# flo-stilz/Audio-Key-Estimation

Hardware: AMD Instinct MI355X
Metric: clips/s (15 s @ 22.05 kHz), HIP CQT + PitchClassNet forward (higher is better)
Workload: dtype f32 accumulation everywhere; pitch / semitone / layer-0 convolutions: f16 activations x f16 weights (per-channel power-of-two scaled) on MFMA, one product; last layer's pitch-class convolutions and heads: 3-term split-bf16 on MFMA (hi*hi + lo*hi + hi*lo); CQT filter bank: 3-term split-bf16 on MFMA

## Files before the change

### audio-key-estimation_amd/csrc/pcnet.hip

```cpp
#include <algorithm>
#include <cmath>
#include <cstdlib>
#include <cstring>
#include <map>
#include <string>
#include <vector>

#include "common.h"
#include "pcnet_kernels.h"
#include "pcnet_bwd_kernels.h"

using namespace ake_k;

namespace {

constexpr double kBnEps = 1e-5;
constexpr size_t kLdsBudget = 64 * 1024;
constexpr size_t kBfFragsPerConv = 14 * 2 * 64 + 64;

struct TensorSpec {
    std::string name;
    int64_t shape[4];
    int ndim;
};
// ... 2273 lines not shown
                                  "conv_p2p_f16x3_kernel/p2p", nullptr, true)) {
                    sdesc = Src{out, d.out_p, nullptr, 0, 0};
                    continue;
                }
                if ((rc = conv(n->p2p[i][j], train ? n->p2p_t[i][j] : n->p2p[i][j], m + "p2p.layer." + std::to_string(3 * j + 1), 0, sdesc,
                               in_aff, B, P, Ti, true, out, d.out_p, 0, out_aff, "conv_mfma_kernel/p2p")))
                    return rc;
                sdesc = Src{out, d.out_p, nullptr, 0, 0};
                in_aff = out_aff;
            }
            if (fused_fold) {
            } else if (fused_semi) {
                if ((rc = run_fold_max(out, d.out_p, P / 3, B, Ti, cat, ctot, d.prev_pc, s))) return rc;
            } else if (c.stay_sixth && train) {
                const long long total = static_cast<long long>(B) * d.out_p * 12 * Ti;
                ake::ProfScope ps("fold_affine_kernel", s);
                hipLaunchKernelGGL(fold_affine_kernel, dim3(static_cast<unsigned>((total + 255) / 256)), dim3(256), 0, s, out, out_aff, cat, d.out_p, P / 12, Ti,
                                   ctot, d.prev_pc, total);
                identity(b.aff_cat[i] + 3 * d.prev_pc, d.out_p);
            } else if (c.stay_sixth) {
                if ((rc = fold_maps(i, out, d.out_p, P, B, Ti, cat, ctot, d.prev_pc))) return rc;
            } else if ((rc = semi(i, out, out_aff, B, P, Ti, cat, ctot, d.prev_pc, train ? b.aff_cat[i] + 3 * d.prev_pc : nullptr))) return rc;
            if (last) return AKE_OK;
            const float* psrc = cat;
            const float* psrc_aff = train ? b.aff_cat[i] : nullptr;
            int cin = ctot;
            float* pdst = nullptr;
            float* pdst_aff = nullptr;
            if (c.resblock && train) {
                if ((rc = res_stack_train(n->pc2pc_t[i], m + "pc2pc.layer.", 1, Src{psrc, cin, nullptr, 0, 0}, psrc_aff, B, 12, Ti, b.pcst[i], b.aff_pcst[i],
                                          nullptr, 0, "conv_mfma_kernel/pc2pc")))
                    return rc;
                pdst = b.pcst[i].back(); pdst_aff = b.aff_pcst[i].back();
            } else if (c.resblock) {
                if ((rc = res_stack(n->pc2pc[i], 1, Src{psrc, cin, nullptr, 0, 0}, B, 12, Ti, b.pca[i], b.pcb[i], nullptr, 0, "conv_mfma_kernel/pc2pc"))) return rc;
                pdst = b.pca[i];
            }
            for (int j = 0; j < c.conv_layers && !c.resblock; ++j) {
                pdst = train ? b.pcst[i][j] : ((j & 1) ? b.pcb[i] : b.pca[i]);
                pdst_aff = !train ? nullptr : b.aff_pcst[i][j];
                if ((rc = conv(n->pc2pc[i][j], train ? n->pc2pc_t[i][j] : n->pc2pc[i][j], m + "pc2pc.layer." + std::to_string(3 * j + 1), 1,
                               Src{psrc, cin, nullptr, 0, 0}, psrc_aff, B, 12, Ti, true, pdst, d.out_pc, 0, pdst_aff, "conv_mfma_kernel/pc2pc")))
                    return rc;
                psrc = pdst; psrc_aff = pdst_aff; cin = d.out_pc;
            }
            const LayerDims& dn = n->dims[i + 1];
            const int ctn = dn.prev_pc + dn.out_p;
            const int Tn = Ti / tp;
            float* catn = b.cat[i + 1] + (i + 1 == L - 1 ? static_cast<size_t>(c0) * ctn * 12 * Tn : 0);
            time_pool(pdst, pdst_aff, B, d.out_pc, 12, Ti, catn, ctn, 0);
            if (train) identity(b.aff_cat[i + 1], d.out_pc);
            time_pool(out, out_aff, B, d.out_p, P, Ti, b.ppool[i], d.out_p, 0);
            pc_cur = catn; p_cur = b.ppool[i]; cp = d.out_p;
        }
        return AKE_OK;
    }

    int tail(int B, const int64_t* seq, float* key_out, float* tonic_out, float* genre_out) {
        const auto& c = n->cfg;
        const int L = c.num_layers, tp = c.time_pool_size;
        const int i = L - 1;
        const int Ti = b.Tl[i];
        const LayerDims& d = n->dims[i];
        int rc;
        const float* psrc = L == 1 ? b.fold0 : b.cat[i];
        const float* psrc_aff = (train && L > 1) ? b.aff_cat[i] : nullptr;
        int cin = L == 1 ? 1 : d.prev_pc + d.out_p;
        const int cout_default = L == 1 ? c.n_filters : d.out_pc;
        const int cout = cout_default;
        const std::string m = "model." + std::to_string(i) + ".pc2pc.layer.";
        float* pdst = nullptr;
        float* pdst_aff = nullptr;
        const bool pc_bf = !train && pc2pc_uses_bf16(n, i, Ti);
        const bool head_bf = !train && L > 1 && n->final_ch == 16 && c.head_layers >= 2 && n->head_key[0].bf_off >= 0 &&
                             n->head_tonic[0].bf_off >= 0 && b.Tf <= kPcBf16MaxFrames;
        const bool pc_fused = !train && L > 1 && !c.denseblock && pc2pc_fuses(n, i, Ti);
        if (pc_fused) {
            if ((rc = run_pc2pc_fused(n, i, psrc, cin, B, Ti, b.pcf, head_bf ? b.feat_cl : nullptr, s))) return rc;
        } else if (pc_bf) run_nchw_to_cl16(psrc, cin, B, Ti, reinterpret_cast<unsigned short*>(b.pcb[i]), s);
        if (c.resblock && train) {
            if ((rc = res_stack_train(n->pc2pc_t[i], m, 1, Src{psrc, cin, nullptr, 0, 0}, psrc_aff, B, 12, Ti, b.pcst[i], b.aff_pcst[i], nullptr, 0,
                                      L == 1 ? "conv_mfma_kernel/pc2pc0" : "conv_mfma_kernel/pc2pc")))
                return rc;
            pdst = b.pcst[i].back(); pdst_aff = b.aff_pcst[i].back();
        } else if (c.resblock) {
            if ((rc = res_stack(n->pc2pc[i], 1, Src{psrc, cin, nullptr, 0, 0}, B, 12, Ti, b.pca[i], b.pcb[i], nullptr, 0,
                                L == 1 ? "conv_mfma_kernel/pc2pc0" : "conv_mfma_kernel/pc2pc")))
                return rc;
            pdst = b.pca[i];
        }
        if (c.denseblock) {
            float* feat_buf = L == 1 ? b.fold0 : b.cat[i];
            if (train) {
                if ((rc = dense_stack_train(n->dense_pc[i], 1, feat_buf, n->final_ch, cin, B, 12, Ti, b.dn_bott_pc[i], b.dn_aff1_pc[i], b.dn_aff2_pc[i],
                                            L == 1 ? "conv_mfma_kernel/pc2pc0" : "conv_mfma_kernel/pc2pc")))
                    return rc;
            } else if ((rc = dense_stack(n->dense_pc[i], 1, feat_buf, n->final_ch, cin, B, 12, Ti, b.pca[i],
                                         L == 1 ? "conv_mfma_kernel/pc2pc0" : "conv_mfma_kernel/pc2pc")))
                return rc;
            pdst = feat_buf; pdst_aff = nullptr;
        }
        for (int j = 0; j < c.conv_layers && !pc_fused && !c.resblock && !c.denseblock; ++j) {
            pdst = train ? b.pcst[i][j] : ((j & 1) ? b.pcb[i] : b.pca[i]);
            pdst_aff = !train ? nullptr : b.aff_pcst[i][j];
            if (pc_bf) {
                const bool last_conv = j == c.conv_layers - 1;
                const unsigned short* in = reinterpret_cast<const unsigned short*>((j & 1) ? b.pca[i] : b.pcb[i]);
                if ((rc = run_pc_bf16(n, n->pc2pc[i][j], in, B, Ti, true, true, last_conv ? pdst : nullptr,
                                      last_conv ? nullptr : reinterpret_cast<unsigned short*>(pdst), s, "conv_pc_bf16_kernel/pc2pc")))
                    return rc;
                continue;
            }
            if (train && L > 1 && pc_f16x3_ok(n->pc2pc_t[i][j], Ti, true)) {
                const PackedConv& pt = n->pc2pc_t[i][j];
                unsigned short* planes = reinterpret_cast<unsigned short*>(b.pcb[i]);
                run_nchw_to_cl16_f16x2(psrc, cin, B, Ti, psrc_aff, planes, s);
                const int bn = bn_of(m + std::to_string(3 * j + 1));
                if ((rc = run_pc_bf16(n, pt, planes, B, Ti, true, false, pdst, nullptr, s, "conv_pc_f16x3_kernel/pc2pc", nullptr, nullptr, true,
                                      b.stats + 2 * n->bns[bn].ch_off, 2 * n->bn_channels)))
                    return rc;
                finalize_bn(bn, static_cast<double>(B) * 12 * Ti, pdst_aff);
                psrc = pdst; psrc_aff = pdst_aff; cin = cout;
                continue;
            }
            if ((rc = conv(n->pc2pc[i][j], train ? n->pc2pc_t[i][j] : n->pc2pc[i][j], m + std::to_string(3 * j + 1), 1,
                           Src{psrc, cin, nullptr, 0, 0}, psrc_aff, B, 12, Ti, true, pdst, cout, 0, pdst_aff,
                           L == 1 ? "conv_mfma_kernel/pc2pc0" : "conv_mfma_kernel/pc2pc")))
                return rc;
            psrc = pdst; psrc_aff = pdst_aff; cin = cout;
        }
        const float* feat = pdst;
        const float* feat_aff = pdst_aff;
        if (pc_fused) { feat = b.pcf; feat_aff = nullptr; }
        else if (L > 1) {
            const int cout = c.denseblock ? n->final_ch : cout_default;
            time_pool(pdst, pdst_aff, B, cout, 12, Ti, b.pcf, cout, 0);
            feat = b.pcf; feat_aff = nullptr;
        }
        const int Tf = b.Tf;
        struct HeadRun { const std::vector<PackedConv>* ce; const std::vector<PackedConv>* ct; float* hid; float* map; int kind; const char* nm; };
        HeadRun heads[3] = {{&n->head_key, &n->head_key_t, b.hid_k, b.map_k, 1, "key_classifier"},
                            {&n->head_tonic, &n->head_tonic_t, b.hid_t, b.map_t, 1, "tonic_classifier"},
                            {&n->head_genre, &n->head_genre_t, b.hid_g, b.map_g, 2, "genre_classifier"}};
        int Tm = Tf;
        bool head_planes_ready = false;
        int pooled_heads = 0;
        unsigned short* feat_cl = b.feat_cl;
        if (head_bf && !pc_fused) run_nchw_to_cl16(feat, n->final_ch, B, Tf, feat_cl, s);
        const int T1 = Tf - (c.kernel_size - 1), T2 = T1 - (c.kernel_size - 1);
        const bool head1_bf = head_bf && c.head_layers == 2 && n->head_key[1].bf_off >= 0 && n->head_tonic[1].bf_off >= 0 && T2 > 0 &&
                              (12 * ((T2 + 15) / 16) + 15) / 16 <= kHead1MT;
        const bool genre_bf = head1_bf && c.genre && n->head_genre.size() == 2 && n->head_genre[0].bf_off >= 0 && n->head_genre[1].bf_off >= 0 &&
                              n->head_genre[0].kh == 1 && n->head_genre[1].kh == 2;
        if (head1_bf) {
            Head1BfArgs ha;
            std::memset(&ha, 0, sizeof(ha));
            float* maps[3] = {b.map_k, b.map_t, b.map_g};
            float* hids[3] = {b.hid_k, b.hid_t, b.hid_g};
            const PackedConv* c0[3] = {&n->head_key[0], &n->head_tonic[0], genre_bf ? &n->head_genre[0] : nullptr};
            const PackedConv* c1[3] = {&n->head_key[1], &n->head_tonic[1], genre_bf ? &n->head_genre[1] : nullptr};
            const int nh = genre_bf ? 3 : 2;
            for (int h = 0; h < nh; ++h) {
                unsigned short* planes = reinterpret_cast<unsigned short*>(hids[h]);
                if (h == 0 && (rc = run_pc_bf16(n, *c0[0], feat_cl, B, Tf, false, true, nullptr, planes, s, "conv_pc_bf16_kernel/head", c0[1],
                                                reinterpret_cast<unsigned short*>(hids[1]))))
                    return rc;
                if (h == 2 && (rc = run_pc_bf16(n, *c0[h], feat_cl, B, Tf, false, true, nullptr, planes, s, "conv_pc_bf16_kernel/genre_head")))
                    return rc;
                ha.xh[h] = planes; ha.xl[h] = planes + static_cast<long long>(B) * 12 * T1 * 32;
                ha.bfrag[h] = n->bf_frags_dev + c1[h]->bf_off; ha.bias[h] = n->blob_dev + c1[h]->b_off; ha.dst[h] = maps[h];
                ha.KH[h] = c1[h]->kh; ha.circular[h] = c1[h]->kh == 12 ? 1 : 0; ha.H_out[h] = ha.circular[h] ? 12 : 12 - c1[h]->kh + 1;
            }
            ha.T_in = T1; ha.T_out = T2; ha.JB = (T2 + 15) / 16; ha.Tp = 16 * (ha.JB - 1) + 22;
            size_t lds = std::max(static_cast<size_t>(2) * 12 * ha.Tp * 4 * sizeof(uint4), static_cast<size_t>(8) * kHead1MT * 4 * 64 * sizeof(float));
            if (c.local == 0) {
                ha.fin_off = static_cast<int>(lds / sizeof(float));
                lds += static_cast<size_t>(12) * T2 * sizeof(float);
                float* outs[3] = {key_out, tonic_out, genre_out};
                for (int h = 0; h < nh; ++h) ha.pout[h] = outs[h];
                ha.seq = reinterpret_cast<const long long*>(seq);
                ha.n_pool_layers = L - 1; ha.tp = tp; ha.shrink = (c.kernel_size - 1) * c.head_layers; ha.max_pool = c.max_pool; ha.clip0 = 0;
                pooled_heads = nh;
            }
            static ake::DeviceOnce h1_attr;
            if (h1_attr.need()) {
                AKE_HIP_CHECK(hipFuncSetAttribute(reinterpret_cast<const void*>(conv_head1_bf16_kernel), hipFuncAttributeMaxDynamicSharedMemorySize, 150 * 1024));
                h1_attr.mark();
            }
            AKE_REQUIRE(lds <= 150 * 1024, AKE_ERR_UNSUPPORTED, "heads: %d frames do not fit conv_head1_bf16_kernel", T1);
            ake::ProfScope ps("conv_head1_bf16_kernel", s);
            hipLaunchKernelGGL(conv_head1_bf16_kernel, dim3(B, nh), dim3(512), lds, s, ha);
            Tm = T2;
        }
        for (int h = head1_bf ? (genre_bf ? 3 : 2) : 0; h < (c.genre ? 3 : 2); ++h) {
            const float* src = feat;
            const float* src_aff = feat_aff;
            int hc = n->final_ch, Tcur = Tf;
            const size_t hid_half = static_cast<size_t>(B) * 2 * n->final_ch * 12 * Tf;
            for (int j = 0; j < c.head_layers; ++j) {
                const PackedConv& pe = (*heads[h].ce)[j];
                const bool lastj = j == c.head_layers - 1;
                float* dst = lastj ? heads[h].map : (train ? b.hst[h][j] : heads[h].hid + (j & 1) * hid_half);
                float* aff = (!train || lastj) ? nullptr : b.aff_hst[h][j];
                if (head_bf && h < 2 && j == 0) {
                    if ((rc = run_pc_bf16(n, pe, feat_cl, B, Tcur, false, true, dst, nullptr, s, "conv_pc_bf16_kernel/head"))) return rc;
                    src = dst; src_aff = aff; hc = pe.cout; Tcur -= c.kernel_size - 1;
                    continue;
                }
                if (train && j == 0 && !lastj && pc_f16x3_ok((*heads[h].ct)[0], Tcur, false)) {
                    const PackedConv& pt = (*heads[h].ct)[0];
                    if (!head_planes_ready) {
                        run_nchw_to_cl16_f16x2(src, hc, B, Tcur, src_aff, b.feat_cl, s);
                        head_planes_ready = true;
                    }
                    const int bn = bn_of(std::string(heads[h].nm) + ".1");
                    if ((rc = run_pc_bf16(n, pt, b.feat_cl, B, Tcur, false, false, dst, nullptr, s,
                                          h == 2 ? "conv_pc_f16x3_kernel/genre_head" : "conv_pc_f16x3_kernel/head", nullptr, nullptr, true,
                                          b.stats + 2 * n->bns[bn].ch_off, 2 * n->bn_channels)))
                        return rc;
                    const int H_out = heads[h].kind == 2 ? 12 - pt.kh + 1 : 12;
                    finalize_bn(bn, static_cast<double>(B) * H_out * (Tcur - pt.kw + 1), aff);
                    src = dst; src_aff = aff; hc = pe.cout; Tcur -= c.kernel_size - 1;
                    continue;
                }
                if (train && lastj && j > 0 && pe.cout == 1 && pe.kw == 7 && !n->raw_w_off.empty()) {
                    const std::string wn = std::string(heads[h].nm) + "." + std::to_string(3 * j) + (heads[h].kind == 2 ? "" : ".conv2d");
                    const auto wi = n->spec_index.find(wn + ".weight"), bi = n->spec_index.find(wn + ".bias");
                    const size_t lds = (static_cast<size_t>(hc) * 12 * Tcur + static_cast<size_t>(hc) * pe.kh * 7) * sizeof(float);
                    if (wi != n->spec_index.end() && bi != n->spec_index.end() && lds <= 150 * 1024 && Tcur - 6 >= 1) {
                        static ake::DeviceOnce hl_attr;
                        if (hl_attr.need()) {
                            AKE_HIP_CHECK(hipFuncSetAttribute(reinterpret_cast<const void*>(conv_head_last_kernel), hipFuncAttributeMaxDynamicSharedMemorySize, 150 * 1024));
                            hl_attr.mark();
                        }
                        ake::ProfScope ps(h == 2 ? "conv_head_last_kernel/genre" : "conv_head_last_kernel", s);
                        hipLaunchKernelGGL(conv_head_last_kernel, dim3(B), dim3(384), lds, s, src, src_aff, n->blob_dev + n->raw_w_off[wi->second],
                                           n->blob_dev + n->raw_w_off[bi->second], dst, hc, pe.kh, heads[h].kind == 2 ? 0 : 1, Tcur, Tcur - 6);
                        src = dst; src_aff = aff; hc = pe.cout; Tcur -= c.kernel_size - 1;
                        continue;
                    }
                }
                if ((rc = conv(pe, train ? (*heads[h].ct)[j] : pe, lastj ? "" : std::string(heads[h].nm) + "." + std::to_string(3 * j + 1),
                               heads[h].kind, Src{src, hc, nullptr, 0, 0}, src_aff, B, 12, Tcur, false, dst, pe.cout, 0, aff,
                               h == 2 ? "conv_mfma_kernel/genre_head" : "conv_mfma_kernel/head")))
                    return rc;
                src = dst; src_aff = aff; hc = pe.cout; Tcur -= c.kernel_size - 1;
            }
            Tm = Tcur;
        }
        if (c.local > 0) {
            AKE_REQUIRE(Tm >= c.local, AKE_ERR_INVALID, "pcnet --local: %d map frames are fewer than the pooling window %d", Tm, c.local);
            LocalPoolArgs la;
            std::memset(&la, 0, sizeof(la));
            la.maps[0] = b.map_k; la.maps[1] = b.map_t; la.maps[2] = c.genre ? b.map_g : nullptr;
            la.outs[0] = key_out; la.outs[1] = tonic_out; la.outs[2] = genre_out;
            la.Tm = Tm; la.Tq = Tm - c.local + 1; la.W = c.local; la.batch = B;
            ake::ProfScope ps("local_pool_kernel", s);
            hipLaunchKernelGGL(local_pool_kernel, dim3(static_cast<unsigned>((static_cast<long long>(B) * 12 * Tm + 255) / 256), 3), dim3(256), 0, s, la);
            AKE_HIP_CHECK(hipGetLastError());
            return AKE_OK;
        }
        PoolHeadArgs pa;
        std::memset(&pa, 0, sizeof(pa));
        pa.maps[0] = b.map_k; pa.maps[1] = b.map_t; pa.maps[2] = c.genre ? b.map_g : nullptr;
        for (int h = 0; h < pooled_heads; ++h) pa.maps[h] = nullptr;
        if (!pa.maps[0] && !pa.maps[1] && !pa.maps[2]) return AKE_OK;
        pa.outs[0] = key_out; pa.outs[1] = tonic_out; pa.outs[2] = genre_out;
        pa.rows[0] = 12; pa.rows[1] = 12; pa.rows[2] = 11;
        pa.Tm = Tm; pa.seq = reinterpret_cast<const long long*>(seq);
        pa.n_pool_layers = L - 1; pa.tp = tp; pa.shrink = (c.kernel_size - 1) * c.head_layers;
        pa.max_pool = c.max_pool; pa.batch = B; pa.clip0 = 0;
        {
            ake::ProfScope ps("head_pool_kernel", s);
            hipLaunchKernelGGL(head_pool_kernel, dim3((B * 12 + 63) / 64, 3), dim3(64), 0, s, pa);
        }
        AKE_HIP_CHECK(hipGetLastError());
        return AKE_OK;
    }
};

int forward_impl(const ake_pcnet* n, bool train, const float* mel, int batch, int frames, const int64_t* seq_length, float* key_out,
                 float* tonic_out, float* genre_out, float* bn_stats_out, void* workspace, size_t ws_bytes, ake_stream_t stream,
                 bool mel_frames_major = false, bool dry_run = false) {
    AKE_REQUIRE(n && mel && key_out && tonic_out, AKE_ERR_INVALID, "pcnet forward: null argument");
    AKE_REQUIRE(n->finalized, AKE_ERR_STATE, "pcnet: ake_pcnet_finalize has not been called");
    AKE_REQUIRE(train || !n->eval_frags_stale, AKE_ERR_STATE,
                "pcnet: the last weight load was ake_pcnet_load_for_training_f32 (training fragments only): call ake_pcnet_load_from_device_f32 before inference");
    AKE_REQUIRE(batch > 0 && frames > 0, AKE_ERR_INVALID, "pcnet: bad batch/frames");
    AKE_REQUIRE(!n->cfg.genre || genre_out, AKE_ERR_INVALID, "pcnet: genre head enabled but genre_out is null");
    const int chunk = train ? batch : std::min(batch, n->chunk_clips);
    Buffers b;
    int rc = plan_buffers(n, batch, chunk, frames, workspace, &b, train);
    if (rc) return rc;
    AKE_REQUIRE(workspace && ws_bytes >= b.bytes, AKE_ERR_WORKSPACE, "pcnet: workspace %zu < %zu bytes", ws_bytes, b.bytes);
    hipStream_t s = static_cast<hipStream_t>(stream);
    if (train) AKE_HIP_CHECK(hipMemsetAsync(b.stats, 0, sizeof(double) * 2 * n->bn_channels * kStatSlots, s));
    Fwd f{n, b, s, train};
    f.mel_fm = mel_frames_major;
    f.chunk = chunk;
    if (dry_run) {
        const auto& c = n->cfg;
        if (train || c.num_layers != 2 || c.resblock || c.denseblock || c.pc2p_mem || c.p2pc_conv || c.stay_sixth || c.local ||
            batch > chunk || !p2p_uses_f16(n, 1, b.Tl[1]))
            return AKE_ERR_UNSUPPORTED;
        if (!f.layer0_fused(mel, batch, true)) return AKE_ERR_UNSUPPORTED;
        const LayerDims& d = n->dims[1];
        Src sdesc{mel, 1, b.psix[1], d.prev_pc, 36};
// ... 216 lines not shown
```

### audio-key-estimation_amd/csrc/pcnet_kernels.h

```cpp
#pragma once

#include <hip/hip_runtime.h>

namespace ake_k {

constexpr int TW = 4;
constexpr float kSlope = 0.01f;

struct ConvArgs {
    const float* src0;
    const float* src1;
    long long src0_clip_stride, src1_clip_stride;
    int c0, c1, h1;
    int H;
    int T_in;
    int T_out;
    int H_out;
    int py;
    int pad_l;
    int time_circ;
    const float* w;
    const float* bias;
    int cout;
    float* dst;
// ... 1547 lines not shown
                        for (int i = 0; i < 4; i += 2) {
                            const float pv = fmaxf(v[i], v[i + 1]);
                            const int tq = (tq0 + i) >> 1;
                            pooled_c[(co * 12 + y) * Tf + tq] = pv;
                            if (a.fh) {
                                const int e = (y * Tf + tq) * 16 + co;
                                const unsigned int hb = bf16_bits(pv);
                                fh_c[e] = static_cast<unsigned short>(hb);
                                fl_c[e] = static_cast<unsigned short>(bf16_bits(pv - __uint_as_float(hb << 16)));
                            }
                        }
                    }
            }
            }
            }
        }
        __syncthreads();
    }
}

struct Head1BfArgs {
    const unsigned short* xh[3];
    const unsigned short* xl[3];
    const uint4* bfrag[3];
    const float* bias[3];
    float* dst[3];
    int KH[3], H_out[3], circular[3];
    int T_in, T_out, Tp, JB;
    float* pout[3];
    const long long* seq;
    int n_pool_layers, tp, shrink, max_pool, clip0;
    int fin_off;
};

constexpr int kHead1MT = 4;

__global__ __launch_bounds__(512) void conv_head1_bf16_kernel(Head1BfArgs a) {
    extern __shared__ __attribute__((aligned(16))) uint4 lds4[];
    const int clip = blockIdx.x, head = blockIdx.y;
    const int lane = threadIdx.x & 63;
    const int wave = __builtin_amdgcn_readfirstlane(threadIdx.x >> 6);
    const int r16 = lane & 15, q = lane >> 4;
    const int Tp = a.Tp;
    uint4* const pH = lds4;
    uint4* const pL = lds4 + 12 * Tp * 4;
    float* const red = reinterpret_cast<float*>(lds4);
    {
        const long long cbase = static_cast<long long>(clip) * 12 * a.T_in * 4;
        const uint4* gh = reinterpret_cast<const uint4*>(a.xh[head]) + cbase;
        const uint4* gl = reinterpret_cast<const uint4*>(a.xl[head]) + cbase;
        const int n16 = 12 * Tp * 4;
        for (int i = threadIdx.x; i < n16; i += blockDim.x) {
            const int grp = i & 3, pos = i >> 2;
            const int row = pos / Tp, f = pos - row * Tp;
            uint4 vh = make_uint4(0, 0, 0, 0), vl = make_uint4(0, 0, 0, 0);
            if (f < a.T_in) {
                const long long g = (static_cast<long long>(row) * a.T_in + f) * 4 + grp;
                vh = gh[g]; vl = gl[g];
            }
            pH[i] = vh; pL[i] = vl;
        }
    }
    __syncthreads();
    const int HO = a.H_out[head], circ = a.circular[head], nks = a.KH[head] * 22;
    const int Mtot = HO * a.JB;
    const int mtiles = (Mtot + 15) / 16;
    int ay[kHead1MT], af[kHead1MT];
#pragma unroll
    for (int mt = 0; mt < kHead1MT; ++mt) {
        int m = mt * 16 + r16;
        if (m >= Mtot) m = Mtot - 1;
        const int jb = m / HO;
        ay[mt] = m - jb * HO;
        af[mt] = 16 * jb;
    }
    typedef float f32x4c __attribute__((ext_vector_type(4)));
    f32x4c acc[kHead1MT];
#pragma unroll
    for (int mt = 0; mt < kHead1MT; ++mt) acc[mt] = f32x4c{0.f, 0.f, 0.f, 0.f};
    const uint4* __restrict__ bg = a.bfrag[head] + lane;
    constexpr int PF = 3;
    uint4 nbh[PF], nbl[PF];
#pragma unroll
    for (int i = 0; i < PF; ++i) {
        const int kn = wave + 8 * i < nks ? wave + 8 * i : wave;
        nbh[i] = bg[(2 * kn + 0) * 64]; nbl[i] = bg[(2 * kn + 1) * 64];
    }
    for (int ks = wave; ks < nks; ks += 8) {
        const int dy = ks / 22, dxe = ks - dy * 22;
        const bf16x8c bh = __builtin_bit_cast(bf16x8c, nbh[0]);
        const bf16x8c bl = __builtin_bit_cast(bf16x8c, nbl[0]);
#pragma unroll
        for (int i = 0; i + 1 < PF; ++i) { nbh[i] = nbh[i + 1]; nbl[i] = nbl[i + 1]; }
        {
            const int kn = ks + 8 * PF < nks ? ks + 8 * PF : ks;
            nbh[PF - 1] = bg[(2 * kn + 0) * 64]; nbl[PF - 1] = bg[(2 * kn + 1) * 64];
        }
#pragma unroll
        for (int mt = 0; mt < kHead1MT; ++mt) {
            if (mt < mtiles) {
                int row = ay[mt] + dy;
                row -= (circ && row >= 12) ? 12 : 0;
                const int ad = ((row * Tp + af[mt] + dxe) << 2) + q;
                const bf16x8c ah = __builtin_bit_cast(bf16x8c, pH[ad]);
                const bf16x8c al = __builtin_bit_cast(bf16x8c, pL[ad]);
                acc[mt] = __builtin_amdgcn_mfma_f32_16x16x32_bf16(ah, bh, acc[mt], 0, 0, 0);
                acc[mt] = __builtin_amdgcn_mfma_f32_16x16x32_bf16(al, bh, acc[mt], 0, 0, 0);
                acc[mt] = __builtin_amdgcn_mfma_f32_16x16x32_bf16(ah, bl, acc[mt], 0, 0, 0);
            }
        }
    }
    __syncthreads();
#pragma unroll
    for (int mt = 0; mt < kHead1MT; ++mt)
#pragma unroll
        for (int i = 0; i < 4; ++i) red[((wave * kHead1MT + mt) * 4 + i) * 64 + lane] = acc[mt][i];
    __syncthreads();
    if (wave < mtiles) {
        const float bias = a.bias[head][0];
#pragma unroll
        for (int i = 0; i < 4; ++i) {
            float v = bias;
#pragma unroll
            for (int w = 0; w < 8; ++w) v += red[((w * kHead1MT + wave) * 4 + i) * 64 + lane];
            const int m = wave * 16 + 4 * q + i;
            const int jb = m / HO, y = m - jb * HO;
            const int t = 16 * jb + r16;
            if (m < Mtot && t < a.T_out) {
                a.dst[head][(static_cast<long long>(clip) * HO + y) * a.T_out + t] = v;
                if (a.pout[head]) reinterpret_cast<float*>(lds4)[a.fin_off + y * a.T_out + t] = v;
            }
        }
    }
    if (a.pout[head] == nullptr) return;
    __syncthreads();
    if (threadIdx.x < HO) {
        bool use_max = a.max_pool != 0;
        const int L = pool_frames(a.seq, clip, a.T_out, a.n_pool_layers, a.tp, a.shrink, a.clip0, &use_max);
        const float* m = reinterpret_cast<const float*>(lds4) + a.fin_off + threadIdx.x * a.T_out;
        float v;
        if (use_max) {
            v = -INFINITY;
            for (int t = 0; t < L; ++t) v = fmaxf(v, m[t]);
        } else {
            float sum = 0.f;
            for (int t = 0; t < L; ++t) sum += m[t];
            v = sum / static_cast<float>(L > 0 ? L : 0);
        }
        if (head == 0) v = 1.f / (1.f + expf(-v));
        a.pout[head][clip * HO + threadIdx.x] = v;
    }
}

__global__ void pack_head1_bf16_kernel(const float* __restrict__ w, uint4* __restrict__ out, int cin, int KH) {
    const int i = blockIdx.x * blockDim.x + threadIdx.x;
    if (i >= KH * 22 * 64) return;
    const int lane = i & 63, ks = i >> 6;
    const int dy = ks / 22, dxe = ks - dy * 22;
    const int tau = lane & 15, qq = lane >> 4;
    const int dx = dxe - tau;
    unsigned int hi[4] = {0, 0, 0, 0}, lo[4] = {0, 0, 0, 0};
    for (int e = 0; e < 8; ++e) {
        const int ci = 8 * qq + e;
        float v = 0.f;
        if (dx >= 0 && dx < 7 && ci < cin) v = w[(ci * KH + dy) * 7 + dx];
        const unsigned int hb = bf16_bits(v);
        hi[e >> 1] |= hb << (16 * (e & 1));
        lo[e >> 1] |= bf16_bits(v - __uint_as_float(hb << 16)) << (16 * (e & 1));
    }
    out[(2 * ks + 0) * 64 + lane] = make_uint4(hi[0], hi[1], hi[2], hi[3]);
    out[(2 * ks + 1) * 64 + lane] = make_uint4(lo[0], lo[1], lo[2], lo[3]);
}

__global__ void pack_pc_bf16_kernel(const float* __restrict__ w, uint4* __restrict__ out, int cin, int cout, int CO, int NT, int KH) {
    const int i = blockIdx.x * blockDim.x + threadIdx.x;
    if (i >= KH * 4 * NT * 64) return;
    const int lane = i & 63, nt = (i >> 6) % NT, ks = i / (64 * NT);
    const int dy = ks >> 2, p = ks & 3;
    const int co = nt * 16 + (lane & 15), qq = lane >> 4;
    const int c8 = 8 * (qq & 1);
    int dx = 2 * p + (qq >> 1), dyw = dy;
    if (p == 3 && !(KH & 1)) {
        dx = (dy & 1) ? 7 : 6;
        dyw = dy + (qq >> 1);
    }
    unsigned int hi[4] = {0, 0, 0, 0}, lo[4] = {0, 0, 0, 0};
    for (int e = 0; e < 8; ++e) {
        const int ci = c8 + e;
        float v = 0.f;
        if (dx < 7 && ci < cin && co < cout) v = w[((((co / CO) * cin + ci) * KH + dyw) * 7 + dx) * CO + (co % CO)];
        const unsigned int hb = bf16_bits(v);
        const unsigned int lb = bf16_bits(v - __uint_as_float(hb << 16));
        hi[e >> 1] |= hb << (16 * (e & 1));
        lo[e >> 1] |= lb << (16 * (e & 1));
    }
    out[((ks * NT + nt) * 2 + 0) * 64 + lane] = make_uint4(hi[0], hi[1], hi[2], hi[3]);
    out[((ks * NT + nt) * 2 + 1) * 64 + lane] = make_uint4(lo[0], lo[1], lo[2], lo[3]);
}

__global__ void nchw_to_cl16_kernel(const float* __restrict__ src, long long src_clip_stride, int C, int T, unsigned short* __restrict__ xh,
                                    unsigned short* __restrict__ xl, long long npos) {
    const long long i = static_cast<long long>(blockIdx.x) * blockDim.x + threadIdx.x;
    if (i >= npos) return;
    const int t = static_cast<int>(i % T);
    const long long r = i / T;
    const int y = static_cast<int>(r % 12);
    const long long clip = r / 12;
    const float* s = src + clip * src_clip_stride + static_cast<long long>(y) * T + t;
    unsigned int hi[8], lo[8];
#pragma unroll
    for (int k = 0; k < 8; ++k) { hi[k] = 0; lo[k] = 0; }
#pragma unroll
    for (int c = 0; c < 16; ++c) {
        const float v = c < C ? s[static_cast<long long>(c) * 12 * T] : 0.f;
        const unsigned int hb = bf16_bits(v);
        hi[c >> 1] |= hb << (16 * (c & 1));
        lo[c >> 1] |= bf16_bits(v - __uint_as_float(hb << 16)) << (16 * (c & 1));
    }
    uint4* oh = reinterpret_cast<uint4*>(xh) + i * 2;
    uint4* ol = reinterpret_cast<uint4*>(xl) + i * 2;
    oh[0] = make_uint4(hi[0], hi[1], hi[2], hi[3]); oh[1] = make_uint4(hi[4], hi[5], hi[6], hi[7]);
    ol[0] = make_uint4(lo[0], lo[1], lo[2], lo[3]); ol[1] = make_uint4(lo[4], lo[5], lo[6], lo[7]);
}

__global__ void nchw_to_cl16_f16x2_kernel(const float* __restrict__ src, long long src_clip_stride, int C, int T, const float* __restrict__ aff,
                                          unsigned short* __restrict__ xh, unsigned short* __restrict__ xl, long long npos,
                                          const unsigned int* __restrict__ amax) {
    const long long i = static_cast<long long>(blockIdx.x) * blockDim.x + threadIdx.x;
    const float mul = amax ? f16_weight_scale(amax_load(amax)) : 1.f;
    if (i >= npos) return;
    const int t = static_cast<int>(i % T);
    const long long r = i / T;
    const int y = static_cast<int>(r % 12);
    const long long clip = r / 12;
    const float* s = src + clip * src_clip_stride + static_cast<long long>(y) * T + t;
    unsigned int hi[8], lo[8];
#pragma unroll
    for (int k = 0; k < 8; ++k) { hi[k] = 0; lo[k] = 0; }
#pragma unroll
    for (int c = 0; c < 16; ++c) {
        float v = 0.f;
        if (c < C) {
            v = s[static_cast<long long>(c) * 12 * T] * mul;
            if (aff) { v = fmaf(v, aff[3 * c], aff[3 * c + 1]); v = v > 0.f ? v : v * aff[3 * c + 2]; }
        }
        const _Float16 h = static_cast<_Float16>(v);
        hi[c >> 1] |= static_cast<unsigned int>(__builtin_bit_cast(unsigned short, h)) << (16 * (c & 1));
        lo[c >> 1] |= f16_bits((v - static_cast<float>(h)) * kP2pLoScale) << (16 * (c & 1));
    }
    uint4* oh = reinterpret_cast<uint4*>(xh) + i * 2;
    uint4* ol = reinterpret_cast<uint4*>(xl) + i * 2;
    oh[0] = make_uint4(hi[0], hi[1], hi[2], hi[3]); oh[1] = make_uint4(hi[4], hi[5], hi[6], hi[7]);
    ol[0] = make_uint4(lo[0], lo[1], lo[2], lo[3]); ol[1] = make_uint4(lo[4], lo[5], lo[6], lo[7]);
}

struct PcPackJob { const float* w; uint4* out; int cin, cout, CO, NT, KH, dy_rot, ci_off; };
constexpr int kMaxPackJobs = 24;
struct PcPackJobs { int n; PcPackJob j[kMaxPackJobs]; };
struct P2pRawJob { const float* w; uint4* out; int cin_fwd, cout_fwd, transpose_flip; };
struct P2pRawJobs { int n; P2pRawJob j[kMaxPackJobs]; };

__device__ __forceinline__ void pc_weight_scale_body(const float* __restrict__ w, float* __restrict__ inv_scale, int cin, int cout, int CO, int KH, int bx) {
    __shared__ float red[4];
    const int co = bx;
    const int g = co / CO, c = co - g * CO;
    float m = 0.f;
    for (int r = threadIdx.x; r < cin * KH * 7; r += blockDim.x) m = fmaxf(m, fabsf(w[(static_cast<long long>(g) * cin * KH * 7 + r) * CO + c]));
#pragma unroll
    for (int o = 32; o > 0; o >>= 1) m = fmaxf(m, __shfl_xor(m, o));
    if ((threadIdx.x & 63) == 0) red[threadIdx.x >> 6] = m;
    __syncthreads();
    if (threadIdx.x == 0) inv_scale[co] = 1.f / f16_weight_scale(fmaxf(fmaxf(red[0], red[1]), fmaxf(red[2], red[3])));
}
__global__ __launch_bounds__(256) void pc_weight_scale_kernel(const float* __restrict__ w, float* __restrict__ inv_scale, int cin, int cout, int CO, int KH) {
    pc_weight_scale_body(w, inv_scale, cin, cout, CO, KH, blockIdx.x);
}
__global__ __launch_bounds__(256) void pc_weight_scale_jobs_kernel(PcPackJobs js) {
    const PcPackJob& J = js.j[blockIdx.y];
    if (static_cast<int>(blockIdx.x) >= J.cout) return;
    pc_weight_scale_body(J.w, reinterpret_cast<float*>(J.out + J.KH * 4 * J.NT * 2 * 64), J.cin, J.cout, J.CO, J.KH, blockIdx.x);
}

__device__ __forceinline__ void pack_pc_f16x3_body(const float* __restrict__ w, uint4* __restrict__ out, int cin, int cout, int CO, int NT, int KH, int dy_rot,
                                                   int ci_off, int bx) {
    const int i = bx * blockDim.x + threadIdx.x;
    if (i >= KH * 4 * NT * 64) return;
    const int lane = i & 63, nt = (i >> 6) % NT, ks = i / (64 * NT);
    const int dy = ks >> 2, p = ks & 3;
    const int co = nt * 16 + (lane & 15), qq = lane >> 4;
    const int c8 = 8 * (qq & 1);
    int dx = 2 * p + (qq >> 1), dyw = dy;
    if (p == 3 && !(KH & 1)) {
        dx = (dy & 1) ? 7 : 6;
        dyw = dy + (qq >> 1);
    }
    const float sc = co < cout ? 1.f / reinterpret_cast<const float*>(out + KH * 4 * NT * 2 * 64)[co] : 1.f;
    unsigned int hi[4] = {0, 0, 0, 0}, lo[4] = {0, 0, 0, 0};
    for (int e = 0; e < 8; ++e) {
        const int ci = ci_off + c8 + e;
        float v = 0.f;
        if (dx < 7 && ci < cin && co < cout) v = sc * w[((((co / CO) * cin + ci) * KH + (dyw + dy_rot) % KH) * 7 + dx) * CO + (co % CO)];
        const _Float16 hv = static_cast<_Float16>(v);
        hi[e >> 1] |= static_cast<unsigned int>(__builtin_bit_cast(unsigned short, hv)) << (16 * (e & 1));
        lo[e >> 1] |= f16_bits((v - static_cast<float>(hv)) * kP2pLoScale) << (16 * (e & 1));
    }
    out[((ks * NT + nt) * 2 + 0) * 64 + lane] = make_uint4(hi[0], hi[1], hi[2], hi[3]);
// ... 865 lines not shown
```

Baseline: 441,400.

## Fuse both head conv layers and pooling into one kernel per clip-head

Adds heads_fused_kernel, which runs the first head convolution (split-bf16 MFMA, with weight rows streamed into LDS through global_load_lds), writes its LeakyReLU output as bf16 hi/lo planes into LDS, then runs the second head convolution and the time pooling in the same block. This replaces the separate run_pc_bf16 launch plus the head1 kernel and removes the global round trip of the hidden planes. The cost is a large dynamic LDS footprint (up to 150 KB), which may limit occupancy. Grid is segments times batch, with genre either sharing the launch or using its own.

```diff
diff --git a/audio-key-estimation_amd/csrc/pcnet.hip b/audio-key-estimation_amd/csrc/pcnet.hip
--- a/audio-key-estimation_amd/csrc/pcnet.hip
+++ b/audio-key-estimation_amd/csrc/pcnet.hip
@@ -2449,7 +2449,55 @@
                               (12 * ((T2 + 15) / 16) + 15) / 16 <= kHead1MT;
         const bool genre_bf = head1_bf && c.genre && n->head_genre.size() == 2 && n->head_genre[0].bf_off >= 0 && n->head_genre[1].bf_off >= 0 &&
                               n->head_genre[0].kh == 1 && n->head_genre[1].kh == 2;
-        if (head1_bf) {
+        constexpr bool kHeadsGenreOwnLaunch = false;
+        const int TpB = 16 * ((T2 + 15) / 16 - 1) + 22;
+        const size_t hf_lds = std::max({(static_cast<size_t>(2) * 12 * (T1 + 8) * 2 + 2 * 4 * 2 * 2 * 64) * sizeof(uint4),
+                                        static_cast<size_t>(2) * 12 * TpB * 4 * sizeof(uint4),
+                                        static_cast<size_t>(8) * kHead1MT * 4 * 64 * sizeof(float)}) +
+                              static_cast<size_t>(12) * T2 * sizeof(float);
+        const bool heads_fused = head1_bf && pc_fused && !g_keep_taps && c.local == 0 && n->head_key[0].cout == 32 && n->head_tonic[0].cout == 32 &&
+                                 n->head_key[0].kh == 12 && n->head_tonic[0].kh == 12 && n->head_key[1].kh == 12 && n->head_tonic[1].kh == 12 &&
+                                 (!genre_bf || n->head_genre[0].cout == 32) && (12 * T1 + 15) / 16 <= 32 && hf_lds <= 150 * 1024;
+        if (heads_fused) {
+            HeadsFusedArgs ha;
+            std::memset(&ha, 0, sizeof(ha));
+            float* maps[3] = {b.map_k, b.map_t, b.map_g};
+            float* outs[3] = {key_out, tonic_out, genre_out};
+            const std::vector<PackedConv>* hc[3] = {&n->head_key, &n->head_tonic, &n->head_genre};
+            ha.xh = feat_cl; ha.xl = feat_cl + static_cast<long long>(B) * 12 * Tf * 16;
+            for (int h = 0; h < (genre_bf ? 3 : 2); ++h) {
+                const PackedConv& p0 = (*hc[h])[0];
+                const PackedConv& p1 = (*hc[h])[1];
+                ha.bfragA[h] = n->bf_frags_dev + p0.bf_off; ha.biasA[h] = n->blob_dev + p0.b_off; ha.KHA[h] = p0.kh;
+                ha.bfragB[h] = n->bf_frags_dev + p1.bf_off; ha.biasB[h] = n->blob_dev + p1.b_off; ha.KHB[h] = p1.kh;
+                ha.dst[h] = maps[h];
+                ha.pout[h] = outs[h];
+            }
+            ha.batch = B; ha.T_in = Tf; ha.T1 = T1; ha.T2 = T2; ha.TpA = T1 + 8; ha.TpB = TpB; ha.JB = (T2 + 15) / 16;
+            ha.fin_off = static_cast<int>(hf_lds / sizeof(float)) - 12 * T2;
+            ha.seq = reinterpret_cast<const long long*>(seq);
+            ha.n_pool_layers = L - 1; ha.tp = tp; ha.shrink = (c.kernel_size - 1) * c.head_layers; ha.max_pool = c.max_pool; ha.clip0 = 0;
+            static ake::DeviceOnce hf_attr;
+            if (hf_attr.need()) {
+                AKE_HIP_CHECK(hipFuncSetAttribute(reinterpret_cast<const void*>(heads_fused_kernel<3>), hipFuncAttributeMaxDynamicSharedMemorySize, 150 * 1024));
+                AKE_HIP_CHECK(hipFuncSetAttribute(reinterpret_cast<const void*>(heads_fused_kernel<4>), hipFuncAttributeMaxDynamicSharedMemorySize, 150 * 1024));
+                hf_attr.mark();
+            }
+            const bool mt3 = (12 * T1 + 15) / 16 <= 24;
+            auto launch = [&](int h0, int h1, int h2, int nseg, const char* name) {
+                ha.hs[0] = h0; ha.hs[1] = h1; ha.hs[2] = h2;
+                ake::ProfScope ps(name, s);
+                if (mt3) hipLaunchKernelGGL(heads_fused_kernel<3>, dim3(nseg * B), dim3(512), hf_lds, s, ha);
+                else hipLaunchKernelGGL(heads_fused_kernel<4>, dim3(nseg * B), dim3(512), hf_lds, s, ha);
+            };
+            if (!genre_bf) launch(0, 1, 1, 2, "heads_fused_kernel");
+            else if (kHeadsGenreOwnLaunch) {
+                launch(0, 1, 1, 2, "heads_fused_kernel");
+                launch(2, 2, 2, 1, "heads_fused_kernel/genre");
+            } else launch(2, 0, 1, 3, "heads_fused_kernel");
+            pooled_heads = genre_bf ? 3 : 2;
+            Tm = T2;
+        } else if (head1_bf) {
             Head1BfArgs ha;
             std::memset(&ha, 0, sizeof(ha));
             float* maps[3] = {b.map_k, b.map_t, b.map_g};
diff --git a/audio-key-estimation_amd/csrc/pcnet_kernels.h b/audio-key-estimation_amd/csrc/pcnet_kernels.h
--- a/audio-key-estimation_amd/csrc/pcnet_kernels.h
+++ b/audio-key-estimation_amd/csrc/pcnet_kernels.h
@@ -1723,6 +1723,273 @@
     }
 }
 
+struct HeadsFusedArgs {
+    const unsigned short* xh;
+    const unsigned short* xl;
+    const uint4* bfragA[3];
+    const float* biasA[3];
+    const uint4* bfragB[3];
+    const float* biasB[3];
+    float* dst[3];
+    float* pout[3];
+    int KHA[3], KHB[3];
+    int hs[3];
+    int batch;
+    int T_in, T1, T2;
+    int TpA, TpB, JB;
+    const long long* seq;
+    int n_pool_layers, tp, shrink, max_pool, clip0;
+    int fin_off;
+};
+
+template <int MT>
+__global__ __launch_bounds__(512, 4) void heads_fused_kernel(HeadsFusedArgs a) {
+    extern __shared__ __attribute__((aligned(16))) uint4 lds4[];
+#define AKE_HSEL(f) (head == 0 ? a.f[0] : head == 1 ? a.f[1] : a.f[2])
+    const int bid = __builtin_amdgcn_readfirstlane(blockIdx.x);
+    const int seg = (bid >= a.batch ? 1 : 0) + (bid >= 2 * a.batch ? 1 : 0);
+    const int clip = bid - seg * a.batch;
+    const int head = seg == 0 ? a.hs[0] : seg == 1 ? a.hs[1] : a.hs[2];
+    const int lane = threadIdx.x & 63;
+    const int wave = __builtin_amdgcn_readfirstlane(threadIdx.x >> 6);
+    const int r16 = lane & 15, q = lane >> 4;
+    typedef float f32x4c __attribute__((ext_vector_type(4)));
+    constexpr int NT = 2;
+    const int TpB = a.TpB;
+    uint4* const pHB = lds4;
+    uint4* const pLB = lds4 + 12 * TpB * 4;
+    const uint4* __restrict__ bg = AKE_HSEL(bfragB) + lane;
+    const int KHB = AKE_HSEL(KHB);
+    const int nks = KHB * 22;
+    constexpr int PF = 3;
+    uint4 nbh[PF], nbl[PF];
+    {
+        const int Tp = a.TpA;
+        const int KH = AKE_HSEL(KHA);
+        const int Mtot = 12 * a.T1;
+        uint4* const pH = lds4;
+        uint4* const pL = lds4 + 12 * Tp * 2;
+        uint4* const wring = lds4 + 2 * 12 * Tp * 2;
+        constexpr int kRow = 4 * NT * 2 * 64;
+        const uint4* const bfr = AKE_HSEL(bfragA);
+        auto fetch_row = [&](int dyn) {
+            for (int pc = wave; pc < kRow / 64; pc += 8) {
+                const uint4* src = bfr + dyn * kRow + pc * 64 + lane;
+                const unsigned int lds_dst = static_cast<unsigned int>(reinterpret_cast<unsigned long long>(wring + (dyn & 1) * kRow + pc * 64));
+                unsigned int keep;
+                asm volatile("s_mov_b32 %0, m0\n\ts_mov_b32 m0, %2\n\ts_nop 0\n\tglobal_load_lds_dwordx4 %1, off\n\ts_mov_b32 m0, %0"
+                             : "=&s"(keep) : "v"(src), "s"(lds_dst) : "memory");
+            }
+        };
+        fetch_row(0);
+        {
+            const long long cbase = static_cast<long long>(clip) * 12 * a.T_in * 2;
+            const uint4* gh = reinterpret_cast<const uint4*>(a.xh) + cbase;
+            const uint4* gl = reinterpret_cast<const uint4*>(a.xl) + cbase;
+            const int n16 = 12 * Tp * 2;
+            for (int i = threadIdx.x; i < n16; i += 512) {
+                const int half = i & 1, pos = i >> 1;
+                const int row = pos / Tp, f = pos - row * Tp;
+                uint4 vh = make_uint4(0, 0, 0, 0), vl = make_uint4(0, 0, 0, 0);
+                if (f < a.T_in) {
+                    const long long g = (static_cast<long long>(row) * a.T_in + f) * 2 + half;
+                    vh = gh[g]; vl = gl[g];
+                }
+                pH[i] = vh; pL[i] = vl;
+            }
+        }
+        __builtin_amdgcn_s_waitcnt(0x0F70);
+        __syncthreads();
+        const int tile0 = wave * MT;
+        const bool active = tile0 * 16 < Mtot;
+        int ay[MT], at[MT];
+#pragma unroll
+        for (int mt = 0; mt < MT; ++mt) {
+            int m = (tile0 + mt) * 16 + r16;
+            if (m >= Mtot) m = Mtot - 1;
+            ay[mt] = m / a.T1;
+            at[mt] = m - ay[mt] * a.T1;
+        }
+        f32x4c acc[MT][NT];
+#pragma unroll
+        for (int mt = 0; mt < MT; ++mt)
+#pragma unroll
+            for (int nt = 0; nt < NT; ++nt) acc[mt][nt] = f32x4c{0.f, 0.f, 0.f, 0.f};
+        const int dxq = q >> 1, half = q & 1;
+        const bool pair = !(KH & 1);
+        for (int dy = 0; dy < KH; ++dy) {
+            if (dy + 1 < KH) fetch_row(dy + 1);
+            const uint4* const wr = wring + (dy & 1) * kRow + lane;
+            if (active) {
+                int rowoff[MT], rowoff3[MT];
+#pragma unroll
+                for (int mt = 0; mt < MT; ++mt) {
+                    int row = ay[mt] + dy;
+                    row -= row >= 12 ? 12 : 0;
+                    rowoff[mt] = ((row * Tp + at[mt] + dxq) << 1) + half;
+                    int row3 = ay[mt] + dy + dxq;
+                    row3 -= row3 >= 12 ? 12 : 0;
+                    rowoff3[mt] = pair ? ((row3 * Tp + at[mt] + 6) << 1) + half : rowoff[mt] + 12;
+                }
+#pragma unroll
+                for (int p = 0; p < 4; ++p) {
+                    if (p == 3 && pair && (dy & 1)) break;
+                    uint4 bhu[NT], blu[NT], ahu[MT], alu[MT];
+#pragma unroll
+                    for (int nt = 0; nt < NT; ++nt) {
+                        bhu[nt] = wr[((p * NT + nt) * 2 + 0) * 64];
+                        blu[nt] = wr[((p * NT + nt) * 2 + 1) * 64];
+                    }
+#pragma unroll
+                    for (int mt = 0; mt < MT; ++mt) {
+                        ahu[mt] = pH[p == 3 ? rowoff3[mt] : rowoff[mt] + 4 * p];
+                        alu[mt] = pL[p == 3 ? rowoff3[mt] : rowoff[mt] + 4 * p];
+                    }
+#pragma unroll
+                    for (int nt = 0; nt < NT; ++nt) {
+                        const bf16x8c bh = __builtin_bit_cast(bf16x8c, bhu[nt]), bl = __builtin_bit_cast(bf16x8c, blu[nt]);
+#pragma unroll
+                        for (int mt = 0; mt < MT; ++mt) acc[mt][nt] = __builtin_amdgcn_mfma_f32_16x16x32_bf16(__builtin_bit_cast(bf16x8c, ahu[mt]), bh, acc[mt][nt], 0, 0, 0);
+#pragma unroll
+                        for (int mt = 0; mt < MT; ++mt) acc[mt][nt] = __builtin_amdgcn_mfma_f32_16x16x32_bf16(__builtin_bit_cast(bf16x8c, alu[mt]), bh, acc[mt][nt], 0, 0, 0);
+#pragma unroll
+                        for (int mt = 0; mt < MT; ++mt) acc[mt][nt] = __builtin_amdgcn_mfma_f32_16x16x32_bf16(__builtin_bit_cast(bf16x8c, ahu[mt]), bl, acc[mt][nt], 0, 0, 0);
+                    }
+                }
+            }
+            if (dy + 1 < KH) {
+                __builtin_amdgcn_s_waitcnt(0x0F70);
+                __syncthreads();
+            }
+        }
+#pragma unroll
+        for (int i = 0; i < PF; ++i) {
+            const int kn = wave + 8 * i < nks ? wave + 8 * i : wave;
+            nbh[i] = bg[(2 * kn + 0) * 64]; nbl[i] = bg[(2 * kn + 1) * 64];
+        }
+        __syncthreads();
+        unsigned short* const sH = reinterpret_cast<unsigned short*>(pHB);
+        unsigned short* const sL = reinterpret_cast<unsigned short*>(pLB);
+        {
+            const int nz = TpB - a.T1, n16 = 12 * nz * 4;
+            for (int i = threadIdx.x; i < n16; i += 512) {
+                const int grp = i & 3, pos = i >> 2;
+                const int row = pos / nz, f = a.T1 + pos - row * nz;
+                pHB[((row * TpB + f) << 2) + grp] = make_uint4(0, 0, 0, 0);
+                pLB[((row * TpB + f) << 2) + grp] = make_uint4(0, 0, 0, 0);
+            }
+        }
+        if (active) {
+            const float* const bptr = AKE_HSEL(biasA);
+#pragma unroll
+            for (int nt = 0; nt < NT; ++nt) {
+                const int co = nt * 16 + r16;
+                const float bias = bptr[co];
+#pragma unroll
+                for (int mt = 0; mt < MT; ++mt) {
+                    const int m0 = (tile0 + mt) * 16 + 4 * q;
+                    int y = m0 / a.T1, t = m0 - y * a.T1;
+#pragma unroll
+                    for (int i = 0; i < 4; ++i) {
+                        if (m0 + i < Mtot) {
+                            float v = acc[mt][nt][i] + bias;
+                            v = v > 0.f ? v : v * kSlope;
+                            const int idx = (y * TpB + t) * 32 + co;
+                            const unsigned int hb = bf16_bits(v);
+                            sH[idx] = static_cast<unsigned short>(hb);
+                            sL[idx] = static_cast<unsigned short>(bf16_bits(v - __uint_as_float(hb << 16)));
+                        }
+                        if (++t == a.T1) { t = 0; ++y; }
+                    }
+                }
+            }
+        }
+    }
+    __syncthreads();
+    float* const red = reinterpret_cast<float*>(lds4);
+    const int circ = KHB == 12 ? 1 : 0;
+    const int HO = circ ? 12 : 12 - KHB + 1;
+    const int Mtot = HO * a.JB;
+    const int mtiles = (Mtot + 15) / 16;
+    int ay[kHead1MT], af[kHead1MT];
+#pragma unroll
+    for (int mt = 0; mt < kHead1MT; ++mt) {
+        int m = mt * 16 + r16;
+        if (m >= Mtot) m = Mtot - 1;
+        const int jb = m / HO;
+        ay[mt] = m - jb * HO;
+        af[mt] = 16 * jb;
+    }
+    f32x4c acc[kHead1MT];
+#pragma unroll
+    for (int mt = 0; mt < kHead1MT; ++mt) acc[mt] = f32x4c{0.f, 0.f, 0.f, 0.f};
+    for (int ks = wave; ks < nks; ks += 8) {
+        const int dy = ks / 22, dxe = ks - dy * 22;
+        const bf16x8c bh = __builtin_bit_cast(bf16x8c, nbh[0]);
+        const bf16x8c bl = __builtin_bit_cast(bf16x8c, nbl[0]);
+#pragma unroll
+        for (int i = 0; i + 1 < PF; ++i) { nbh[i] = nbh[i + 1]; nbl[i] = nbl[i + 1]; }
+        {
+            const int kn = ks + 8 * PF < nks ? ks + 8 * PF : ks;
+            nbh[PF - 1] = bg[(2 * kn + 0) * 64]; nbl[PF - 1] = bg[(2 * kn + 1) * 64];
+        }
+#pragma unroll
+        for (int mt = 0; mt < kHead1MT; ++mt) {
+            if (mt < mtiles) {
+                int row = ay[mt] + dy;
+                row -= (circ && row >= 12) ? 12 : 0;
+                const int ad = ((row * TpB + af[mt] + dxe) << 2) + q;
+                const bf16x8c ah = __builtin_bit_cast(bf16x8c, pHB[ad]);
+                const bf16x8c al = __builtin_bit_cast(bf16x8c, pLB[ad]);
+                acc[mt] = __builtin_amdgcn_mfma_f32_16x16x32_bf16(ah, bh, acc[mt], 0, 0, 0);
+                acc[mt] = __builtin_amdgcn_mfma_f32_16x16x32_bf16(al, bh, acc[mt], 0, 0, 0);
+                acc[mt] = __builtin_amdgcn_mfma_f32_16x16x32_bf16(ah, bl, acc[mt], 0, 0, 0);
+            }
+        }
+    }
+    __syncthreads();
+#pragma unroll
+    for (int mt = 0; mt < kHead1MT; ++mt)
+#pragma unroll
+        for (int i = 0; i < 4; ++i) red[((wave * kHead1MT + mt) * 4 + i) * 64 + lane] = acc[mt][i];
+    __syncthreads();
+    if (wave < mtiles) {
+        const float bias = AKE_HSEL(biasB)[0];
+        float* const dst = AKE_HSEL(dst);
+#pragma unroll
+        for (int i = 0; i < 4; ++i) {
+            float v = bias;
+#pragma unroll
+            for (int w = 0; w < 8; ++w) v += red[((w * kHead1MT + wave) * 4 + i) * 64 + lane];
+            const int m = wave * 16 + 4 * q + i;
+            const int jb = m / HO, y = m - jb * HO;
+            const int t = 16 * jb + r16;
+            if (m < Mtot && t < a.T2) {
+                dst[(static_cast<long long>(clip) * HO + y) * a.T2 + t] = v;
+                reinterpret_cast<float*>(lds4)[a.fin_off + y * a.T2 + t] = v;
+            }
+        }
+    }
+    __syncthreads();
+    if (threadIdx.x < HO) {
+        bool use_max = a.max_pool != 0;
+        const int L = pool_frames(a.seq, clip, a.T2, a.n_pool_layers, a.tp, a.shrink, a.clip0, &use_max);
+        const float* m = reinterpret_cast<const float*>(lds4) + a.fin_off + threadIdx.x * a.T2;
+        float v;
+        if (use_max) {
+            v = -INFINITY;
+            for (int t = 0; t < L; ++t) v = fmaxf(v, m[t]);
+        } else {
+            float sum = 0.f;
+            for (int t = 0; t < L; ++t) sum += m[t];
+            v = sum / static_cast<float>(L > 0 ? L : 0);
+        }
+        if (head == 0) v = 1.f / (1.f + expf(-v));
+        AKE_HSEL(pout)[clip * HO + threadIdx.x] = v;
+    }
+#undef AKE_HSEL
+}
+
 __global__ void pack_head1_bf16_kernel(const float* __restrict__ w, uint4* __restrict__ out, int cin, int KH) {
     const int i = blockIdx.x * blockDim.x + threadIdx.x;
     if (i >= KH * 22 * 64) return;
```

After: 470,700, median of 6. 1.07x the previous value.
